# madsjulia/GeostatInversion.jl

Measured on AMD Instinct MI355X. Metric: randSVD GB/s + top-k singular-value rel-err, n=1e6 rank=256, higher is better.
Workload: dtype f64

## Files before the change

geostatinversion.jl_amd/build.py:

```python
import os
import shutil
import subprocess
import sys
from concurrent.futures import ThreadPoolExecutor

HERE = os.path.dirname(os.path.abspath(__file__))
CSRC = os.path.join(HERE, "csrc")
OBJ = os.path.join(HERE, "build")
LIB = os.path.join(HERE, "libgsi_hip.so")
SOURCES = ["gemm_f64.hip", "gemm_f64_gen1.hip", "syrk_f64.hip", "panel_lu_leaf.hip", "panel_lu_blocks.hip", "panel_lu_streamed.hip", "panel_lu_sharded.hip", "panel_qr.hip", "cholqr.hip", "lowrank_power.hip", "jacobi_svd.hip", "misc.hip", "lsqr_dev.hip", "pointcov_gemm.hip", "fft_cov.hip", "fft_gridcov_plan.hip", "fftrf_sample.hip", "fftrf_interp.hip", "pcga_forward.hip", "chol_saddle.hip",
           "hip_backend.hip", "hip_comm.hip", "pipeline.cpp", "api.cpp"]
HEADERS = ["backend.hpp", "hip_backend.hpp", "hip_common.hpp", "panel_lu_dev.hpp", "pipeline.hpp", "lsqr_state.hpp", "pointcov.hpp", "pointcov_gen.hpp", "host_staging.hpp", "gemm_f64_kernel.inc.hpp", "fft_line.hpp", "jacobi_sched.hpp", "fwd_plan.hpp", "fftrf_points.hpp", "saddle_host.hpp", "../../include/gsi_hip.h"]
CXXFLAGS = ["-O3", "-std=c++17", "-fPIC", "--offload-arch=gfx950", "-Wall", "-Wno-unused-function",
            "-Wno-unused-result", "-Wno-unused-value"]
RESOURCE_FLAG = "-Rpass-analysis=kernel-resource-usage"
_RES_KEYS = {"TotalSGPRs": "sgprs", "VGPRs": "vgprs", "AGPRs": "agprs", "ScratchSize [bytes/lane]": "scratch_bytes_per_lane",
             "Occupancy [waves/SIMD]": "occupancy_waves_per_simd", "SGPRs Spill": "sgpr_spills", "VGPRs Spill": "vgpr_spills",
             "LDS Size [bytes/block]": "lds_bytes_per_block", "Dynamic Stack": "dynamic_stack"}


def parse_resource_remarks(text):
    out, cur = {}, None
    for line in text.splitlines():
        if "remark:" not in line or "[-Rpass-analysis=kernel-resource-usage]" not in line:
            continue
        body = line.split("remark:", 1)[1].replace("[-Rpass-analysis=kernel-resource-usage]", "").strip()
        if ":" not in body:
            continue
        key, val = [x.strip() for x in body.rsplit(":", 1)]
        if key == "Function Name":
            cur = out.setdefault(val, {})
        elif cur is not None and key in _RES_KEYS:
            cur[_RES_KEYS[key]] = (val == "True") if key == "Dynamic Stack" else int(val)
    return out


def hipcc_version():
    r = subprocess.run([_hipcc(), "--version"], capture_output=True, text=True)
    lines = [ln.strip() for ln in r.stdout.splitlines() if ln.strip()]
    return "; ".join(lines[:2])


def kernel_resources():
    import json
    res = {}
    for src in SOURCES:
        if not src.endswith(".hip"):
            continue
        path = os.path.join(OBJ, src.replace(".", "_") + ".resources.json")
        if not os.path.exists(path):
            raise RuntimeError(f"{path} missing: run build() (it recompiles sources whose resource record is absent)")
        for name, r in json.load(open(path)).items():
            res[name] = dict(r, source=src)
    return res


def _hipcc():
    for cand in (shutil.which("hipcc"), "/opt/rocm/bin/hipcc"):
        if cand and os.path.exists(cand):
            return cand
    raise RuntimeError("hipcc not found: libgsi_hip.so cannot be built (there is no CPU fallback)")


# ... 54 lines not shown
```

geostatinversion.jl_amd/csrc/api.cpp:

```cpp
#include <cmath>
#include <cstdlib>
#include <cstring>
#include <memory>
#include <new>
#include <string>
#include <vector>
#include "../../include/gsi_hip.h"
#include "pipeline.hpp"
#include "pointcov.hpp"
#include "fftrf_points.hpp"

using namespace gsi;

struct gsi_ctx {
  Context c;
};
struct gsi_op {
  Operator op;
};
struct gsi_mat {
  gsi_ctx* ctx;
  Buf buf;
  int64_t rows, cols;
  int refs = 1;
// ... 952 lines not shown
  return guarded([&] {
    REQUIRE(ctx && Y && Q_out, "NULL argument");
    REQUIRE(m >= 1 && l >= 1 && l <= m, "qr_thinQ: need 1 <= l <= m (tall panel)");
    Backend* be = ctx->c.be.get();
    Buf P(be, (size_t)m * l), R(be, (size_t)l * l);
    be->upload2d(P.p, m, Y, m, m, l);
    {
      ScopedPhase ph(be, PH_QR);
      be->qr_thinQ(P.p, m, l, m, R.p);
    }
    be->download2d(Q_out, m, P.p, m, m, l);
    if (R_out) be->download2d(R_out, l, R.p, l, l, l);
    check_async_errors(ctx->c);
  });
}

int gsi_svd_tall(gsi_ctx* ctx, const double* W, int64_t n, int64_t l, double* V_out, double* S_out) {
  return guarded([&] {
    REQUIRE(ctx && W && V_out && S_out, "NULL argument");
    REQUIRE(n >= 1 && l >= 1 && l <= n, "svd_tall: need 1 <= l <= n");
    Backend* be = ctx->c.be.get();
    Buf Wd(be, (size_t)n * l), V(be, (size_t)n * l), S(be, (size_t)l);
    be->upload2d(Wd.p, n, W, n, n, l);
    svd_tall(ctx->c, Wd.p, n, l, -1, V.p, S.p);
    be->download2d(V_out, n, V.p, n, n, l);
    be->download2d(S_out, l, S.p, l, l, 1);
    check_async_errors(ctx->c);
  });
}

int gsi_gemm(gsi_ctx* ctx, int trans, int64_t m, int64_t l, int64_t k, double alpha, const double* A,
             int64_t lda, const double* B, int64_t ldb, double* C, int64_t ldc) {
  return guarded([&] {
    REQUIRE(ctx && A && B && C, "NULL argument");
    REQUIRE(m >= 1 && l >= 1 && k >= 1, "bad shape");
    const int64_t ar = trans ? k : m, ac = trans ? m : k;
    REQUIRE(lda >= ar && ldb >= k && ldc >= m, "leading dimension too small");
    Backend* be = ctx->c.be.get();
    Buf Ad(be, (size_t)ar * ac), Bd(be, (size_t)k * l), Cd(be, (size_t)m * l);
    be->upload2d(Ad.p, ar, A, lda, ar, ac);
    be->upload2d(Bd.p, k, B, ldb, k, l);
    if (trans) be->gemm_tn(m, l, k, alpha, Ad.p, ar, Bd.p, k, 0.0, Cd.p, m);
    else be->gemm_nn(m, l, k, alpha, Ad.p, ar, Bd.p, k, 0.0, Cd.p, m);
    be->download2d(C, ldc, Cd.p, m, m, l);
    check_async_errors(ctx->c);
  });
}

int gsi_gemm_view(gsi_ctx* ctx, int form, int trans, int64_t m, int64_t l, int64_t k, double alpha, double beta,
                  const double* A, int64_t lda, int64_t a_off, const double* B, int64_t ldb, int64_t b_off, double* C,
                  int64_t ldc, int64_t c_off, int64_t m_full, int64_t r0, int64_t* plan_out) {
  return guarded([&] {
    REQUIRE(ctx && A && C && plan_out, "NULL argument");
    REQUIRE(form >= 0 && form <= 3, "gemm_view: form is 0 (gemm), 1 (syrk upper), 2 (trmm upper) or 3 (NN row block)");
    REQUIRE(m >= 1 && l >= 1 && k >= 1, "bad shape");
    REQUIRE(form == 1 || B, "NULL argument");
    REQUIRE(form == 0 || (alpha == 1.0 && beta == 0.0), "gemm_view: forms 1 to 3 compute C = op(A) B (alpha 1, beta 0)");
    REQUIRE(form == 0 || !trans, "gemm_view: trans belongs to form 0");
    REQUIRE(form != 1 || m == l, "gemm_view: form 1 is the l x l product A'A (m == l)");
    REQUIRE(form != 3 || (r0 >= 0 && r0 + m <= m_full), "gemm_view: row block outside the full product");
    const bool tn = trans || form == 1;
    const int64_t ar = (form == 3) ? m_full : (tn ? k : m), ac = tn ? m : k;
    const int64_t crows = (form == 3) ? m_full : m;
    REQUIRE(lda >= ar && ldc >= crows && (form == 1 || ldb >= k), "leading dimension too small");
    REQUIRE(a_off >= 0 && b_off >= 0 && c_off >= 0, "negative offset");
    Backend* be = ctx->c.be.get();
    const size_t na = (size_t)a_off + (size_t)lda * (size_t)ac, nc = (size_t)c_off + (size_t)ldc * (size_t)l;
    const size_t nb = (form == 1) ? 1 : (size_t)b_off + (size_t)ldb * (size_t)l;
    Buf Ad(be, na), Bd(be, nb), Cd(be, nc);
    be->fill_bytes(Ad.p, 0xFF, na);
    be->fill_bytes(Bd.p, 0xFF, nb);
    be->upload2d(Ad.p + a_off, lda, A, ar, ar, ac);
    if (form != 1) be->upload2d(Bd.p + b_off, ldb, B, k, k, l);
    be->upload2d(Cd.p, (int64_t)nc, C, (int64_t)nc, (int64_t)nc, 1);
    be->gemm_view(form, trans != 0, m, l, k, alpha, Ad.p + a_off, lda, Bd.p + b_off, ldb, beta, Cd.p + c_off, ldc, m_full, r0,
                  plan_out);
    be->download2d(C, (int64_t)nc, Cd.p, (int64_t)nc, (int64_t)nc, 1);
    check_async_errors(ctx->c);
  });
}

namespace {
void pcga_params_impl(Context& c, const double* Zdev, int64_t n, int64_t K, const double* s, const double* X,
                      double delta, double* out) {
  Backend* be = c.be.get();
  Buf O(be, (size_t)n * (K + 3)), sv(be, (size_t)n), Xv(be, (size_t)n);
  be->upload2d(sv.p, n, s, n, n, 1);
  be->upload2d(Xv.p, n, X, n, n, 1);
  be->pcga_params(Zdev, n, K, sv.p, Xv.p, delta, O.p);
  be->download2d(out, n, O.p, n, n, K + 3);
}
void pcga_update_impl(Context& c, const double* Zdev, int64_t n, int64_t K, const double* X, double beta_bar,
                      const double* etas, int64_t nobs, const double* xi_bar, double* s_out) {
  Backend* be = c.be.get();
  Buf E(be, (size_t)nobs * K), xb(be, (size_t)nobs), w(be, (size_t)K), sd(be, (size_t)n), Xd(be, (size_t)n);
  be->upload2d(E.p, nobs, etas, nobs, nobs, K);
  be->upload2d(xb.p, nobs, xi_bar, nobs, nobs, 1);
  be->upload2d(Xd.p, n, X, n, n, 1);
  be->gemm_tn(K, 1, nobs, 1.0, E.p, nobs, xb.p, nobs, 0.0, w.p, K);
  be->scal_copy(n, beta_bar, Xd.p, sd.p);
  be->gemm_nn(n, 1, K, 1.0, Zdev, n, w.p, K, 1.0, sd.p, n);
  be->download2d(s_out, n, sd.p, n, n, 1);
}
}

int gsi_pcga_params(gsi_ctx* ctx, const double* Z, int64_t n, int64_t K, const double* s, const double* X,
                    double delta, double* out) {
  return guarded([&] {
    REQUIRE(ctx && Z && s && X && out, "NULL argument");
    REQUIRE(n >= 1 && K >= 1, "bad shape");
    Buf Zd(ctx->c.be.get(), (size_t)n * K);
// ... 315 lines not shown
```

geostatinversion.jl_amd/csrc/hip_backend.hip:

```cpp
#include <dlfcn.h>
#include <algorithm>
#include <cmath>
#include <cstdlib>
#include <cstring>
#include <mutex>
#include <map>
#include <memory>
#include <set>
#include <vector>
#include "hip_backend.hpp"
#include "hip_common.hpp"
#include "host_staging.hpp"
#include "fftrf_points.hpp"

namespace gsi {

namespace {

struct DevBuf {
  void* p = nullptr;
  size_t bytes = 0;
  bool pooled = false;
};

// ... 256 lines not shown
        HIP_CHECK(hipEventSynchronize(e1));
        float ms = 0.f;
        HIP_CHECK(hipEventElapsedTime(&ms, e0, e1));
        if (ms > 0.f) best[dir] = std::max(best[dir], (double)bytes / (ms * 1e-3) / 1e9);
      }
    *h2d_gbs = best[0];
    *d2h_gbs = best[1];
  }
  void upload2d_end(void* handle) override {
    if (!handle) return;
    try {
      static_cast<HostStager*>(handle)->end();
    } catch (const std::exception& e) {
      throw Error(GSI_ERR_HIP, e.what());
    }
  }
  void copy2d(double* dst, int64_t ldd, const double* src, int64_t lds, int64_t rows, int64_t cols) override {
    if (rows <= 0 || cols <= 0) return;
    bind();
    HIP_CHECK(hipMemcpy2DAsync(dst, ldd * sizeof(double), src, lds * sizeof(double), rows * sizeof(double),
                               cols, hipMemcpyDeviceToDevice, st_));
  }
  void fill_zero(double* p, size_t count) override {
    bind();
    HIP_CHECK(hipMemsetAsync(p, 0, count * sizeof(double), st_));
  }
  void sync() override {
    bind();
    HIP_CHECK(hipStreamSynchronize(st_));
    if (st2_) HIP_CHECK(hipStreamSynchronize(st2_));
  }

  void gemm_nn(int64_t m, int64_t l, int64_t k, double alpha, const double* A, int64_t lda, const double* B,
               int64_t ldb, double beta, double* C, int64_t ldc) override {
    bind();
    double* ws = gemm_ws(hipk::gemm_workspace_doubles(m, l, k));
    hipk::gemm_f64(st_, false, m, l, k, alpha, A, lda, B, ldb, beta, C, ldc, ws);
    check_launch("gemm_nn");
  }
  void gemm_nn_rowblock(int64_t m_full, int64_t r0, int64_t mb, int64_t l, int64_t k, const double* A, int64_t lda,
                        const double* B, int64_t ldb, double* C, int64_t ldc) override {
    bind();
    double* ws = gemm_ws(hipk::gemm_rowblock_workspace_doubles(m_full, mb, l, k));
    hipk::gemm_f64_nn_rowblock(st_, m_full, r0, mb, l, k, A, lda, B, ldb, C, ldc, ws);
    check_launch("gemm_nn_rowblock");
  }
  void gemm_tn(int64_t m, int64_t l, int64_t k, double alpha, const double* A, int64_t lda, const double* B,
               int64_t ldb, double beta, double* C, int64_t ldc) override {
    bind();
    double* ws = gemm_ws(hipk::gemm_workspace_doubles(m, l, k));
    hipk::gemm_f64(st_, true, m, l, k, alpha, A, lda, B, ldb, beta, C, ldc, ws);
    check_launch("gemm_tn");
  }
  void gemm_view(int form, bool trans, int64_t m, int64_t l, int64_t k, double alpha, const double* A, int64_t lda,
                 const double* B, int64_t ldb, double beta, double* C, int64_t ldc, int64_t m_full, int64_t r0,
                 int64_t* plan8) override {
    bind();
    hipk::GemmPlan p = {0, 0, 0, 0, 0, 0, 0, 0};
    if (form == 0) {
      double* ws = gemm_ws(hipk::gemm_workspace_doubles(m, l, k));
      hipk::gemm_f64(st_, trans, m, l, k, alpha, A, lda, B, ldb, beta, C, ldc, ws, &p);
    } else if (form == 1) {
      double* ws = gemm_ws(hipk::gemm_syrk_workspace_doubles(l, k));
      hipk::gemm_f64_syrk_upper(st_, l, k, A, lda, C, ldc, ws, &p);
    } else if (form == 2) {
      double* ws = gemm_ws(hipk::gemm_workspace_doubles(m, l, k));
      hipk::gemm_f64_trmm_upper(st_, m, l, k, A, lda, B, ldb, C, ldc, ws, &p);
    } else {
      double* ws = gemm_ws(hipk::gemm_rowblock_workspace_doubles(m_full, m, l, k));
      hipk::gemm_f64_nn_rowblock(st_, m_full, r0, m, l, k, A, lda, B, ldb, C, ldc, ws, &p);
    }
    check_launch("gemm_view");
    const int64_t out[8] = {p.nt, p.nchunks, p.xmode, p.wide, p.nsplit, p.persistent, p.grid_x, p.active};
    for (int i = 0; i < 8; ++i) plan8[i] = out[i];
  }
  void fill_bytes(double* p, int byte, size_t count) override {
    bind();
    HIP_CHECK(hipMemsetAsync(p, byte, count * sizeof(double), st_));
  }
  void gemm_nn_gridcov(int64_t m, int64_t l, int64_t k, const double* tab, int64_t nx, int64_t ny, int64_t roff,
                       int64_t koff, const double* B, int64_t ldb, double* C, int64_t ldc) override {
    bind();
    double* ws = gemm_ws(hipk::gemm_workspace_doubles(m, l, k));
    hipk::gemm_f64_gridcov(st_, m, l, k, tab, nx, ny, roff, koff, B, ldb, C, ldc, ws);
    check_launch("gemm_nn_gridcov");
  }

  void gemm_nn_pointcov(int64_t m, int64_t l, int64_t k, const double* pts, int d, int kind, double ell, double sigma2,
                        double nugget, int64_t roff, int64_t koff, const double* B, int64_t ldb, double* C,
                        int64_t ldc) override {
    bind();
    if (m <= 0 || l <= 0 || k <= 0) return;
    const int64_t npts = std::max(roff + m, koff + k);
    Scratch p4(this, (size_t)4 * npts);
    hipk::pointcov_pad_points(st_, pts, d, npts, hipk::pointcov_point_scale(kind, 1.0 / ell), p4.p);
    double* ws = gemm_ws(hipk::gemm_pointcov_workspace_doubles(m, l, k));
    Scratch xpack(this);
    const size_t xdoubles = hipk::gemm_pointcov_pack_doubles(m, l, k);
    if (xdoubles > 0) xpack.try_alloc(xdoubles);
    hipk::gemm_f64_pointcov(st_, m, l, k, p4.p, npts, d, kind, sigma2, nugget, roff, koff, B, ldb, C, ldc, ws, xpack.p);
    check_launch("gemm_nn_pointcov (in-loader generator)");
  }

  struct FftCov {
    int64_t N[3], M[3]; Scratch lam, W; int nb_max;
    explicit FftCov(HipBackend* be) : lam(be), W(be) {}
  };
  std::unique_ptr<FftCov> fftcov_new_plan(const int64_t N[3], int fftrf, bool* reembed, int* dims) {
    std::unique_ptr<FftCov> p(new FftCov(this));
    int64_t Mtot = 1;
    int d = 0;
    for (int a = 0; a < 3; ++a) { p->N[a] = 1; p->M[a] = 1; }
    *reembed = false;
    for (int a = 0; a < 3; ++a) {
      if (N[a] < 1) throw Error(GSI_ERR_ARG, "fft covariance: grid dimensions must be >= 1");
      if (N[a] == 1) continue;
      p->N[d] = N[a]; p->M[d] = hipk::fft_embed_size(N[a]);
      if (fftrf && p->M[d] != 2 * N[a]) *reembed = true;
      if (p->M[d] > 8192) throw Error(GSI_ERR_ARG, "fft covariance: at most 4096 grid points per axis (a line must fit LDS)");
      Mtot *= p->M[d];
      ++d;
    }
    if (Mtot >= ((int64_t)1 << 31))
// ... 485 lines not shown
  bool lowrank_tail(const double* Sm, int64_t lds, int64_t n, int64_t N, const double* G, const double* T, int64_t l,
                    int64_t K, double c, double* Z, int64_t ldz, double* Sv, double* scratch, size_t scratch_doubles) override {
    bind();
    if (!cholqr_gate(n, l) || l < 1 || l > 384 || l > N - 1 || K < 1 || K > l || N > 4096) return false;
    static const double ov_env = [] {
      const char* e = getenv("GSI_LOWRANK_TAIL_OVERLAP");
      if (e == nullptr || e[0] == 0) return -1.0;
      const double v = atof(e);
      return (v > 0.0 && v < 1.0) ? v : 0.0;
    }();
    static const int reserve = [] {
      const char* e = getenv("GSI_LOWRANK_TAIL_RESERVE_CUS");
      const int v = e ? atoi(e) : TAIL_RESERVE_CUS;
      return (v >= 8 && (v & 7) == 0) ? v : TAIL_RESERVE_CUS;
    }();
    const size_t Nl = ((size_t)N * l + 7) & ~(size_t)7, ll = ((size_t)l * l + 7) & ~(size_t)7;
    Scratch buf(this, 3 * Nl + 12 * ll);
    const int cap = std::max(8, ((ncus_ - reserve) / 8) * 8);
    int64_t nf = 0;
    if (ov_env != 0.0) {
      nf = (int64_t)((ov_env > 0.0 ? ov_env : TAIL_OVERLAP_FRACTION) * (double)n) / 128 * 128;
      if (nf >= n) nf = (n - 1) / 128 * 128;
    }
    double* A0 = buf.p;
    double* A1 = A0 + Nl;
    double* P = A1 + Nl;
    double* Gr[4];
    for (int i = 0; i < 4; ++i) Gr[i] = P + Nl + (size_t)i * ll;
    double* X[4];
    for (int i = 0; i < 4; ++i) X[i] = P + Nl + (size_t)(4 + i) * ll;
    double* R = P + Nl + 8 * ll;
    double* Rf = R + ll;
    double* U = Rf + ll;
    double* Mm = U + ll;
    size_t gmax = hipk::gemm_workspace_doubles(N, l, N);
    gmax = std::max(gmax, hipk::gemm_workspace_doubles(l, l, N));
    gmax = std::max(gmax, hipk::gemm_workspace_doubles(N, l, l));
    gmax = std::max(gmax, hipk::gemm_workspace_doubles(l, l, l));
    gmax = std::max(gmax, hipk::gemm_workspace_doubles(N, K, l));
    gmax = std::max(gmax, hipk::gemm_workspace_doubles(n, K, N));
    if (nf >= 128) {
      hipk::GemmPlan plan = {0, 0, 0, 0, 0, 0, 0, 0};
      const bool takes = hipk::gemm_f64_nn_capped(st_, nf, l, N, Sm, lds, A1, N, A1, nf, cap, true, &plan);
      if (!takes || (ov_env < 0.0 && plan.persistent == 0)) nf = 0;
    } else {
      nf = 0;
    }
    Scratch own(this, (nf > 0 && (scratch == nullptr || scratch_doubles < (size_t)nf * (size_t)l)) ? (size_t)nf * (size_t)l : 0);
    double* Yf = (nf > 0) ? (own.p != nullptr ? own.p : scratch) : nullptr;
    if (nf > 0) gmax = std::max(gmax, hipk::gemm_workspace_doubles(nf, K, l));
    double* ws = gemm_ws(gmax + 64);
    SideJoin side(this);
    auto round = [&](const double* M, int i, bool check) {
      hipk::gemm_f64(st_, false, N, l, N, 1.0, G, N, M, N, 0.0, P, N, ws);
      hipk::gemm_f64(st_, true, l, l, N, 1.0, M, N, P, N, 0.0, Gr[i], l, ws);
      (void)hipk::cq_gram_round(st_, Gr[i], l, X[i], check, flags_ + FLAG_CHOLQR);
    };
    phase_begin(PH_QR);
    HIP_CHECK(hipMemsetAsync(flags_ + FLAG_CHOLQR, 0, sizeof(int32_t), st_));
    hipk::scal_copy(st_, (int64_t)N * l, c, T, A0);
    round(A0, 0, false);
    hipk::gemm_f64(st_, false, N, l, l, 1.0, A0, N, X[0], l, 0.0, A1, N, ws);
    round(A1, 1, true);
    hipk::scal_copy(st_, (int64_t)N * l, c, P, A0);
    round(A0, 2, false);
    hipk::gemm_f64(st_, false, N, l, l, 1.0, A0, N, X[2], l, 0.0, A1, N, ws);
    round(A1, 3, true);
    check_launch("lowrank_tail");
    if (nf > 0) {
      side.fork();
      (void)hipk::gemm_f64_nn_capped(st2_, nf, l, N, Sm, lds, A1, N, Yf, nf, cap);
      check_launch("lowrank_tail (side product)");
    }
    if (read_flag(FLAG_CHOLQR) != 0) {
      side.join();
      phase_end(PH_QR);
      return false;
    }
    hipk::tri_product(st_, Gr[3], Gr[2], l, R);
    hipk::gemm_f64(st_, false, l, l, l, 1.0, R, l, X[1], l, 0.0, Rf, l, ws);
    phase_end(PH_QR);
    n_cholqr_ += 2;
    phase_begin(PH_SVD);
    svd_small(Rf, l, U, Sv);
    hipk::scale_cols_sqrt(st_, U, l, Sv, K);
    phase_end(PH_SVD);
    phase_begin(PH_SMALL_GEMM);
    hipk::gemm_f64(st_, false, l, K, l, 1.0, X[3], l, U, l, 0.0, Mm, l, ws);
    hipk::gemm_f64(st_, false, N, K, l, 1.0, A1, N, Mm, l, 0.0, A0, N, ws);
    if (nf > 0) {
      side.join();
      hipk::gemm_f64(st_, false, nf, K, l, 1.0, Yf, nf, Mm, l, 0.0, Z, ldz, ws);
      hipk::gemm_f64_nn_rowblock(st_, n, nf, n - nf, K, N, Sm, lds, A0, N, Z, ldz, ws);
      ++n_tail_overlaps_;
    } else {
      hipk::gemm_f64(st_, false, n, K, N, 1.0, Sm, lds, A0, N, 0.0, Z, ldz, ws);
    }
    if (K < l) HIP_CHECK(hipMemsetAsync(Z + (size_t)K * ldz, 0, sizeof(double) * ((size_t)(l - K - 1) * ldz + n), st_));
    check_launch("lowrank_tail");
    phase_end(PH_SMALL_GEMM);
    return true;
  }
  bool lowrank_power_step(const double* Sm, int64_t lds, int64_t n, int64_t N, const double* G, const double* T,
                          const int32_t* ipiv, const double* L, int64_t ldl, int64_t l, double c, double* Tn) override {
    bind();
    static const bool trace = (getenv("GSI_LOWRANK_POWER_TRACE") != nullptr);
    constexpr int64_t NSAMPLE = 256;
    constexpr int NPARTS = 128;
    constexpr double CHECK_MAX = 1e-8;
    if (l < 1 || l > 384 || N < 1 || N > 4096 || n < 2 * l || n >= ((int64_t)1 << 31)) return false;
    const int64_t ns = std::min<int64_t>(NSAMPLE, n - l), nchk = l + ns;
    auto up8 = [](int64_t x) { return (x + 7) & ~(int64_t)7; };
    const int64_t o_chk = up8(2 * l), o_sm = o_chk + up8(nchk), nr = o_sm + 2 * l, ldr = up8(nr);
    const size_t nidx = (size_t)(2 * ldr + nchk);
    const size_t ll = (size_t)up8(l * l), Nl = (size_t)up8(N * l);
    Scratch buf(this, 2 * ll + Nl + (size_t)ldr * (size_t)N + (size_t)ldr * (size_t)l + nidx + NPARTS + 2);
    double* Mp = buf.p;
    double* Ut = Mp + ll;
    double* C = Ut + ll;
    double* R = C + Nl;
    double* E = R + (size_t)ldr * N;
    int64_t* idx_dev = reinterpret_cast<int64_t*>(E + (size_t)ldr * l);
    double* part = reinterpret_cast<double*>(idx_dev + nidx);
    int32_t* verdict = reinterpret_cast<int32_t*>(part + NPARTS);
    const int64_t me = o_chk + nchk;
    size_t gmax = hipk::gemm_workspace_doubles(l, l, N);
    gmax = std::max(gmax, hipk::gemm_workspace_doubles(me, l, N));
    gmax = std::max(gmax, hipk::gemm_workspace_doubles(N, l, N));
    gmax = std::max(gmax, hipk::gemm_workspace_doubles(N, l, 2 * l));
    double* ws = gemm_ws(gmax + 64);
    struct Verdict { double parts[NPARTS]; int32_t v[4]; };
    if (pin_power_ == nullptr) HIP_CHECK(hipHostMalloc(&pin_power_, sizeof(Verdict), hipHostMallocDefault));
    hipk::lr_compose(st_, ipiv, flags_ + FLAG_LU_INFO, n, l, nchk, o_chk, o_sm, ldr, idx_dev, idx_dev + ldr, idx_dev + 2 * ldr, verdict);
    hipk::lr_gather_rows(st_, Sm, lds, N, idx_dev, idx_dev + ldr, nr, R, ldr);
    hipk::gemm_f64(st_, false, l, l, N, 1.0, R + o_chk, ldr, T, N, 0.0, Mp, l, ws);
    hipk::lr_solve_u(st_, L, ldl, Mp, l, c, Ut);
    hipk::lr_solve_c(st_, Ut, l, T, N, c, C);
    hipk::gemm_f64(st_, false, me, l, N, 1.0, R, ldr, C, N, 0.0, E, ldr, ws);
    hipk::lr_check_rows(st_, E + o_chk, ldr, L, ldl, idx_dev + 2 * ldr, nchk, l, part, NPARTS);
    hipk::gemm_f64(st_, false, N, l, N, 1.0, G, N, C, N, 0.0, Tn, N, ws);
    hipk::gemm_f64(st_, true, N, l, 2 * l, 1.0, R + o_sm, ldr, E, ldr, 1.0, Tn, N, ws);
    check_launch("lowrank_power_step");
    const Verdict* h = static_cast<const Verdict*>(pin_power_);
    HIP_CHECK(hipMemcpyAsync(pin_power_, part, sizeof(Verdict), hipMemcpyDeviceToHost, st_));
    HIP_CHECK(hipStreamSynchronize(st_));
    double mx = 0.0;
    bool finite = true;
    for (int p = 0; p < NPARTS; ++p) {
      if (!std::isfinite(h->parts[p])) finite = false;
      else mx = std::max(mx, h->parts[p]);
    }
    if (!finite) mx = INFINITY;
    if (trace) fprintf(stderr, "lowrank_power_step: n %lld N %lld l %lld, %lld moved rows, check max |(P S) C - L| = %.3e\n",
                       (long long)n, (long long)N, (long long)l, (long long)h->v[2], mx);
    if (h->v[0] != 0 || h->v[1] != 0) return false;
    return finite && mx <= CHECK_MAX;
  }
  static constexpr int64_t SPLIT_MAX_L1 = 192;
  struct SplitWs { int32_t* piv; int32_t* verdict1; int32_t* verdict2; int64_t* idx1; int64_t o_chk, o_sm, ldr; };
  static int64_t up8(int64_t x) { return (x + 7) & ~(int64_t)7; }
  SplitWs split_ws(int64_t l1) {
    SplitWs w;
    w.o_chk = up8(2 * l1); w.o_sm = w.o_chk + up8(l1); w.ldr = up8(w.o_sm + 2 * l1);
    grow(ws_split_, 2048 + sizeof(int64_t) * (size_t)(2 * up8(5 * SPLIT_MAX_L1 + 16) + SPLIT_MAX_L1));
    char* base = (char*)ws_split_.p;
    w.piv = (int32_t*)base;
    w.verdict1 = (int32_t*)(base + 1536 + 64);
    w.verdict2 = w.verdict1 + 4;
    w.idx1 = (int64_t*)(base + 2048);
    return w;
  }
  bool lu2_resident_ok() const {
    static const bool tall_first = (getenv("GSI_LU_TALL") != nullptr && getenv("GSI_LU_TALL")[0] == '1');
    return !tall_first && !lu2_lost_ && ranks_sharing_device_ <= 1;
  }
  bool lu2_takes(int64_t m, hipk::Lu2Work* w) {
    return lu2_resident_ok() && hipk::lu2_config(m, ncus_, &w->bs, &w->rpt, &w->grid) && lu2_fits(w->bs, w->rpt, w->grid);
  }
  bool lowrank_split_ok(int64_t n, int64_t N, int64_t l, int64_t l1) override {
    bind();
    if (l1 < 1 || l1 > SPLIT_MAX_L1 || l <= l1 || l > 2 * l1 || l - l1 < 8 || l > 384 || N < 1 || N > 4096 || n < 2 * l ||
        n >= ((int64_t)1 << 31))
      return false;
    hipk::Lu2Work w;
    return lu2_takes(n, &w) && lu2_takes(n - l1, &w);
  }
  void lowrank_split_schur(const double* Sm, int64_t lds, int64_t n, int64_t N, const double* T, const int32_t* ipiv1,
                           const double* P, int64_t ldp, int64_t l, int64_t l1, double c, double* Tt) override {
    bind();
    const int64_t l2 = l - l1;
    const SplitWs w = split_ws(l1);
    const size_t l1l = (size_t)up8(l1 * l), Nl1 = (size_t)up8(N * l1);
    Scratch buf(this, (size_t)up8(l1) * (size_t)N + 2 * l1l + 8 + Nl1);
    double* R = buf.p;
    double* Mp = R + (size_t)up8(l1) * N;
    double* Ut11 = Mp + l1l;
    double* U12 = Ut11 + (size_t)up8(l1 * l1);
    double* C1 = Mp + 2 * l1l + 8;
    size_t gmax = hipk::gemm_workspace_doubles(l1, l, N);
    gmax = std::max(gmax, hipk::gemm_workspace_doubles(N, l2, l1));
    double* ws = gemm_ws(gmax + 64);
    int64_t* src = w.idx1, * sub = w.idx1 + w.ldr, * chk = w.idx1 + 2 * w.ldr;
    hipk::lr_compose(st_, ipiv1, flags_ + FLAG_LU_INFO, n, l1, l1, w.o_chk, w.o_sm, w.ldr, src, sub, chk, w.verdict1);
    hipk::lr_pivots(st_, ipiv1, l1, 0, w.piv);
    hipk::lr_gather_rows(st_, Sm, lds, N, src + w.o_chk, sub + w.o_chk, l1, R, up8(l1));
    hipk::gemm_f64(st_, false, l1, l, N, 1.0, R, up8(l1), T, N, 0.0, Mp, l1, ws);
    hipk::lr_solve_u12(st_, P, ldp, Mp, l1, l, c, Ut11, U12);
    hipk::lr_solve_c(st_, Ut11, l1, T, N, c, C1);
    hipk::scal_copy(st_, N * l2, c, T + (size_t)N * l1, Tt);
    hipk::gemm_f64(st_, false, N, l2, l1, -1.0, C1, N, U12, l1, 1.0, Tt, N, ws);
    check_launch("lowrank_split_schur");
  }
  void lowrank_split_rows(double* P, int64_t ldp, int64_t n, int64_t l, int64_t l1) override {
    bind();
    (void)n;
    const int64_t l2 = l - l1;
    const SplitWs w = split_ws(l1);
    Scratch tmp(this, (size_t)(2 * l1) * (size_t)l2);
    hipk::lr_move_rows(st_, P + (size_t)l1 * ldp, ldp, l2, w.idx1, w.idx1 + w.ldr, w.verdict1, 2 * l1, tmp.p, 2 * l1, l1);
    check_launch("lowrank_split_rows");
  }
  void lowrank_split_join(double* P, int64_t ldp, int64_t n, int64_t l, int64_t l1, const int32_t* ipiv2,
                          int32_t** ipiv) override {
    bind();
    const int64_t l2 = l - l1;
    const SplitWs w = split_ws(l1);
    const int64_t ldr = up8(4 * l2);
    Scratch buf(this, (size_t)(2 * ldr + 8) + (size_t)(2 * l2) * (size_t)l1);
    int64_t* src = reinterpret_cast<int64_t*>(buf.p), * sub = src + ldr, * chk = sub + ldr;
    double* tmp = buf.p + 2 * ldr + 8;
    hipk::lr_compose(st_, ipiv2, flags_ + FLAG_LU_INFO, n - l1, l2, 0, 2 * l2, 2 * l2, ldr, src, sub, chk, w.verdict2);
    hipk::lr_pivots(st_, ipiv2, l2, l1, w.piv + l1);
    hipk::lr_move_rows(st_, P + l1, ldp, l1, src, sub, w.verdict2, 2 * l2, tmp, 2 * l2, 0);
    check_launch("lowrank_split_join");
    *ipiv = w.piv;
  }
  void lowrank_split_undo() override {
    bind();
    hipk::lr_forget_zero_pivot(st_, flags_ + FLAG_LU_INFO);
    check_launch("lowrank_split_undo");
  }
  void svd_small(double* G, int64_t l, double* U, double* S) override {
    bind();
    if (l > 5000) throw Error(GSI_ERR_ARG, "sketch width l = K+p > 5000 is not supported by the LDS-resident block Jacobi SVD");
    grow(ws_svd_, sizeof(double) * (l + 8) + 64 + sizeof(int32_t) * hipk::SVD_SCHED_INTS);
    hipk::SvdWork w;
    w.norms = (double*)ws_svd_.p;
    w.pairs = (int32_t*)((char*)ws_svd_.p + sizeof(double) * (l + 8) + 64);
    w.rotcount = flags_ + FLAG_SVD_ROTATIONS;
    const int sw = hipk::svd_small(st_, G, l, U, S, w);
    last_svd_sweeps_ = sw < 0 ? -sw : sw;
    if (sw < 0) ++n_svd_cap_hits_;
    check_launch("svd_small");
  }
  void chol_upper(double* B, int64_t j) override {
    bind();
    if (j > 2048) throw Error(GSI_ERR_ARG, "chol_upper: j too large");
    hipk::chol_upper(st_, B, j, flags_ + FLAG_CHOL_INFO);
    check_launch("chol_upper");
  }
  void trsm_right_upper(double* F, int64_t m, int64_t j, int64_t ldf, const double* C) override {
    bind();
    hipk::trsm_right_upper(st_, F, m, j, ldf, C);
// ... 509 lines not shown
```

geostatinversion.jl_amd/csrc/hip_common.hpp:

```cpp
#pragma once
#include <hip/hip_runtime.h>
#include <atomic>
#include <cstdint>
#include <cstddef>
#include "pointcov.hpp"

namespace gsi { struct FwdProduct; }

namespace gsi { namespace hipk {

inline bool first_use_on_this_device(std::atomic<uint64_t>& mask) {
  int dev = 0;
  if (hipGetDevice(&dev) != hipSuccess || dev < 0 || dev > 63) return true;
  const uint64_t bit = (uint64_t)1 << dev;
  return (mask.fetch_or(bit, std::memory_order_acq_rel) & bit) == 0;
}

struct GemmPlan { int64_t nt, nchunks, xmode, wide, nsplit, persistent, grid_x, active; };
size_t gemm_workspace_doubles(int64_t M, int64_t L, int64_t K);
void gemm_f64(hipStream_t st, bool transA, int64_t M, int64_t L, int64_t K, double alpha, const double* A,
              int64_t lda, const double* B, int64_t ldb, double beta, double* C, int64_t ldc, double* ws,
              GemmPlan* plan = nullptr);
bool gemm_f64_nn_capped(hipStream_t st, int64_t M, int64_t L, int64_t K, const double* A, int64_t lda, const double* B,
                        int64_t ldb, double* C, int64_t ldc, int max_grid, bool query_only = false, GemmPlan* plan = nullptr);
size_t gemm_rowblock_workspace_doubles(int64_t M_full, int64_t mb, int64_t L, int64_t K);
void gemm_f64_nn_rowblock(hipStream_t st, int64_t M_full, int64_t r0, int64_t mb, int64_t L, int64_t K, const double* A,
                          int64_t lda, const double* B, int64_t ldb, double* C, int64_t ldc, double* ws,
                          GemmPlan* plan = nullptr);
size_t gemm_syrk_workspace_doubles(int64_t l, int64_t m);
size_t syrk_upper_workspace_doubles(int64_t l, int64_t m);
bool syrk_full_from_upper(hipStream_t st, int64_t l, int64_t m, const double* Y, int64_t ld, double* G, int64_t ldg, double* ws);
bool trmm_upper_tall(hipStream_t st, int64_t m, int64_t l, const double* A, int64_t lda, const double* X, int64_t ldx, double* C,
                     int64_t ldc);
void gemm_f64_syrk_upper(hipStream_t st, int64_t l, int64_t m, const double* A, int64_t lda, double* C, int64_t ldc,
                         double* ws, GemmPlan* plan = nullptr);
void gemm_f64_trmm_upper(hipStream_t st, int64_t M, int64_t L, int64_t K, const double* A, int64_t lda, const double* B,
                         int64_t ldb, double* C, int64_t ldc, double* ws, GemmPlan* plan = nullptr);
void gemm_f64_gridcov(hipStream_t st, int64_t M, int64_t L, int64_t K, const double* tab, int64_t nx, int64_t ny,
                      int64_t roff, int64_t koff, const double* B, int64_t ldb, double* C, int64_t ldc, double* ws);

void gemm_f64_pointcov(hipStream_t st, int64_t M, int64_t L, int64_t K, const double* pts4, int64_t npts, int d, int kind,
                       double sigma2, double nugget, int64_t roff, int64_t koff, const double* B, int64_t ldb, double* C,
                       int64_t ldc, double* ws, double* xpack);
double pointcov_point_scale(int kind, double inv_ell);
bool gemm_f64_pointcov_wide(hipStream_t st, int64_t M, int64_t L, int64_t K, const double* pts4, int64_t npts, int d, int kind,
                            double sigma2, double nugget, int64_t roff, int64_t koff, const double* B, int64_t ldb, double* C,
                            int64_t ldc, double* ws, double* xpack);
size_t gemm_pointcov_workspace_doubles(int64_t M, int64_t L, int64_t K);
size_t gemm_pointcov_pack_doubles(int64_t M, int64_t L, int64_t K);
int gemm_choose_split(int64_t nwg, int64_t K);
void gemm_splitk_reduce(hipStream_t st, int64_t M, int64_t L, int nsplit, const double* slabs, double* C, int64_t ldc);
void pointcov_pad_points(hipStream_t st, const double* pts, int d, int64_t n, double scale, double* out4);
int64_t fft_embed_size(int64_t N);
size_t fft_plan_doubles(const int64_t M[3]);
void fft_spectrum(hipStream_t st, double* lam, double* part64, const int64_t M[3], double beta, int fftrf);
void fft_cos_matrix(hipStream_t st, double* out, int64_t rows, int64_t cols, int64_t period, bool weighted);
void fft_lines_layout(hipStream_t st, const double* nat, double* out, const int64_t M[3]);
void fft_spectrum_natural(hipStream_t st, double* lam, const int64_t M[3], double beta, int fftrf);
void fft_finish_plan(hipStream_t st, double* lam, double* part64, const int64_t M[3]);
void fft_plan_twiddles(hipStream_t st, double* lam, const int64_t M[3]);
void fft_lag_table(hipStream_t st, double* cp, double* cm, const int64_t N[3], int kind, const double inv_ell[3], double cs,
                   double sn, double sigma2);
void fft_even_odd_split(hipStream_t st, double* cp, double* cm, int64_t total);
void fft_sin_matrix(hipStream_t st, double* out, int64_t rows, int64_t cols, int64_t period);
void fft_subtract(hipStream_t st, double* a, const double* b, int64_t total);
void fft_finish_plan_lags(hipStream_t st, double* lam, const int64_t M[3], double nugget);
void fft_cov_apply(hipStream_t st, const int64_t N[3], const int64_t M[3], const double* lam, double2* W, int nb_max,
                   int64_t l, const double* X, int64_t ldx, double* Y, int64_t ldy);

struct FftrfGeom { int d; int64_t A[3], L[3], P[3]; int blue[3]; int64_t Mtot, n; };
void fftrf_geometry(int ndims, const int64_t* N, FftrfGeom* g);
size_t fftrf_plan_doubles(const FftrfGeom& g);
size_t fftrf_field_doubles(const FftrfGeom& g);
void fftrf_plan(hipStream_t st, const FftrfGeom& g, double* plan);
void fftrf_sample(hipStream_t st, const FftrfGeom& g, const double* plan, double* ws, int64_t fs, int nb, double k0, double dk,
                  double beta, double* dst, int64_t ldd, int64_t row0, int64_t nloc);
void fftrf_interp(hipStream_t st, int d, const int32_t* base, const double* frac, int64_t m, int64_t s1, int64_t s2,
                  const double* V, int64_t v_fs, int nb, double* dst, int64_t ldd);

constexpr int LU2_LEAF = 8;
constexpr int LU2_NB = 64;
// ... 166 lines not shown
```

Baseline: 1762.

## Add small-tile MFMA f64 GEMM for small products in low-rank power and QR

Adds a dedicated f64 GEMM kernel with 32x32 tiles and register prefetch, built on 16x16x4 f64 MFMA. It is used for small products (m up to 4096, l up to 384, small k) in the CholeskyQR tail, the power step and the split Schur paths. The aim is to cut launch and tiling overhead and raise occupancy on small operands, where the general GEMM's large tiles and workspace split waste work. It also exposes the kernel as gemm_view form 4 and adds an environment switch to disable it. The risk is lower throughput than the tuned general kernel on shapes near the thresholds.

```diff
diff --git a/geostatinversion.jl_amd/build.py b/geostatinversion.jl_amd/build.py
--- a/geostatinversion.jl_amd/build.py
+++ b/geostatinversion.jl_amd/build.py
@@ -8,7 +8,7 @@
 CSRC = os.path.join(HERE, "csrc")
 OBJ = os.path.join(HERE, "build")
 LIB = os.path.join(HERE, "libgsi_hip.so")
-SOURCES = ["gemm_f64.hip", "gemm_f64_gen1.hip", "syrk_f64.hip", "panel_lu_leaf.hip", "panel_lu_blocks.hip", "panel_lu_streamed.hip", "panel_lu_sharded.hip", "panel_qr.hip", "cholqr.hip", "lowrank_power.hip", "jacobi_svd.hip", "misc.hip", "lsqr_dev.hip", "pointcov_gemm.hip", "fft_cov.hip", "fft_gridcov_plan.hip", "fftrf_sample.hip", "fftrf_interp.hip", "pcga_forward.hip", "chol_saddle.hip",
+SOURCES = ["gemm_f64.hip", "gemm_f64_gen1.hip", "gemm_f64_small.hip", "syrk_f64.hip", "panel_lu_leaf.hip", "panel_lu_blocks.hip", "panel_lu_streamed.hip", "panel_lu_sharded.hip", "panel_qr.hip", "cholqr.hip", "lowrank_power.hip", "jacobi_svd.hip", "misc.hip", "lsqr_dev.hip", "pointcov_gemm.hip", "fft_cov.hip", "fft_gridcov_plan.hip", "fftrf_sample.hip", "fftrf_interp.hip", "pcga_forward.hip", "chol_saddle.hip",
            "hip_backend.hip", "hip_comm.hip", "pipeline.cpp", "api.cpp"]
 HEADERS = ["backend.hpp", "hip_backend.hpp", "hip_common.hpp", "panel_lu_dev.hpp", "pipeline.hpp", "lsqr_state.hpp", "pointcov.hpp", "pointcov_gen.hpp", "host_staging.hpp", "gemm_f64_kernel.inc.hpp", "fft_line.hpp", "jacobi_sched.hpp", "fwd_plan.hpp", "fftrf_points.hpp", "saddle_host.hpp", "../../include/gsi_hip.h"]
 CXXFLAGS = ["-O3", "-std=c++17", "-fPIC", "--offload-arch=gfx950", "-Wall", "-Wno-unused-function",
diff --git a/geostatinversion.jl_amd/csrc/api.cpp b/geostatinversion.jl_amd/csrc/api.cpp
--- a/geostatinversion.jl_amd/csrc/api.cpp
+++ b/geostatinversion.jl_amd/csrc/api.cpp
@@ -1028,11 +1028,14 @@
                   int64_t ldc, int64_t c_off, int64_t m_full, int64_t r0, int64_t* plan_out) {
   return guarded([&] {
     REQUIRE(ctx && A && C && plan_out, "NULL argument");
-    REQUIRE(form >= 0 && form <= 3, "gemm_view: form is 0 (gemm), 1 (syrk upper), 2 (trmm upper) or 3 (NN row block)");
+    REQUIRE(form >= 0 && form <= 4,
+            "gemm_view: form is 0 (gemm), 1 (syrk upper), 2 (trmm upper), 3 (NN row block) or 4 (small product, m_full = max workgroups)");
     REQUIRE(m >= 1 && l >= 1 && k >= 1, "bad shape");
     REQUIRE(form == 1 || B, "NULL argument");
-    REQUIRE(form == 0 || (alpha == 1.0 && beta == 0.0), "gemm_view: forms 1 to 3 compute C = op(A) B (alpha 1, beta 0)");
-    REQUIRE(form == 0 || !trans, "gemm_view: trans belongs to form 0");
+    REQUIRE(form == 0 || form == 4 || (alpha == 1.0 && beta == 0.0), "gemm_view: forms 1 to 3 compute C = op(A) B (alpha 1, beta 0)");
+    REQUIRE(form == 0 || form == 4 || !trans, "gemm_view: trans belongs to forms 0 and 4");
+    REQUIRE(form != 4 || (m_full >= 0 && m_full < ((int64_t)1 << 30) && (r0 == 0 || r0 == 32 || r0 == 64)),
+            "gemm_view: form 4 takes max workgroups (0: no cap) in m_full and the tile rows (0: the launcher's, 32, 64) in r0");
     REQUIRE(form != 1 || m == l, "gemm_view: form 1 is the l x l product A'A (m == l)");
     REQUIRE(form != 3 || (r0 >= 0 && r0 + m <= m_full), "gemm_view: row block outside the full product");
     const bool tn = trans || form == 1;
diff --git a/geostatinversion.jl_amd/csrc/gemm_f64_small.hip b/geostatinversion.jl_amd/csrc/gemm_f64_small.hip
--- /dev/null
+++ b/geostatinversion.jl_amd/csrc/gemm_f64_small.hip
@@ -0,0 +1,206 @@
+#include "hip_common.hpp"
+
+namespace gsi { namespace hipk {
+
+namespace {
+typedef double sp_double4 __attribute__((ext_vector_type(4)));
+constexpr int SP_THREADS = 256, SP_BN = 32, SP_BK = 32, SP_LDK = SP_BK + 2;
+constexpr int64_t SP_MAX_LD = (int64_t)1 << 20;
+
+template <int BM, bool TA>
+struct SpGeom {
+  static constexpr int WM = BM / 16, WN = 4 / WM, NACC = SP_BN / 16 / WN;
+  static constexpr int NA = BM * SP_BK / SP_THREADS, NB = SP_BN * SP_BK / SP_THREADS;
+  static constexpr int LDA_S = TA ? SP_LDK : BM + 16;
+  static constexpr int A_DOUBLES = TA ? BM * SP_LDK : SP_BK * (BM + 16);
+  static constexpr int B_DOUBLES = SP_BN * SP_LDK;
+  static constexpr int PF = BM == 32 ? 4 : 2;
+  static constexpr int KPASS = SP_THREADS / BM;
+};
+
+template <int NA, int NB>
+__device__ __forceinline__ void sp_load(double (&ra)[NA], double (&rb)[NB], const char* Ab, const char* Bb,
+                                        const uint32_t (&oa)[NA], const uint32_t (&ob)[NB]) {
+#pragma unroll
+  for (int i = 0; i < NA; ++i) ra[i] = *reinterpret_cast<const double*>(Ab + oa[i]);
+#pragma unroll
+  for (int i = 0; i < NB; ++i) rb[i] = *reinterpret_cast<const double*>(Bb + ob[i]);
+}
+
+template <int BM, bool TA, int NA, int NB>
+__device__ __forceinline__ void sp_load_tail(double (&ra)[NA], double (&rb)[NB], const char* Ab, const char* Bb, int64_t lda,
+                                             int64_t ldb, int mrem, int lrem, int krem) {
+  using G = SpGeom<BM, TA>;
+  const int t = threadIdx.x;
+#pragma unroll
+  for (int i = 0; i < NA; ++i) {
+    const int k = TA ? (t & 31) : t / BM + G::KPASS * i, r = min(TA ? (t >> 5) + 8 * i : t % BM, mrem - 1), kc = min(k, krem - 1);
+    const double v = *reinterpret_cast<const double*>(Ab + 8 * (TA ? kc + r * lda : r + kc * lda));
+    ra[i] = k < krem ? v : 0.0;
+  }
+#pragma unroll
+  for (int i = 0; i < NB; ++i) {
+    const int k = t & 31, c = min((t >> 5) + 8 * i, lrem - 1), kc = min(k, krem - 1);
+    const double v = *reinterpret_cast<const double*>(Bb + 8 * (kc + c * ldb));
+    rb[i] = k < krem ? v : 0.0;
+  }
+}
+
+template <int BM, bool TA, int NA, int NB>
+__device__ __forceinline__ void sp_stage(const double (&ra)[NA], const double (&rb)[NB], double* As, double* Bs) {
+  using G = SpGeom<BM, TA>;
+  const int t = threadIdx.x;
+  double* pa = TA ? As + (t >> 5) * SP_LDK + (t & 31) : As + (t / BM) * G::LDA_S + t % BM;
+  double* pb = Bs + (t >> 5) * SP_LDK + (t & 31);
+#pragma unroll
+  for (int i = 0; i < G::NA; ++i) pa[i * (TA ? 8 * SP_LDK : G::KPASS * G::LDA_S)] = ra[i];
+#pragma unroll
+  for (int i = 0; i < G::NB; ++i) pb[i * 8 * SP_LDK] = rb[i];
+}
+
+template <int BM, bool TA, int NACC>
+__device__ __forceinline__ void sp_mma(sp_double4 (&acc)[NACC], const double* as, const double* bs) {
+  using G = SpGeom<BM, TA>;
+  double a[SP_BK / 4], b[SP_BK / 4][NACC];
+#pragma unroll
+  for (int ks = 0; ks < SP_BK / 4; ++ks) {
+    a[ks] = as[TA ? ks * 4 : ks * 4 * G::LDA_S];
+#pragma unroll
+    for (int j = 0; j < NACC; ++j) b[ks][j] = bs[j * 16 * SP_LDK + ks * 4];
+  }
+#pragma unroll
+  for (int ks = 0; ks < SP_BK / 4; ++ks) {
+#pragma unroll
+    for (int j = 0; j < NACC; ++j) acc[j] = __builtin_amdgcn_mfma_f64_16x16x4f64(b[ks][j], a[ks], acc[j], 0, 0, 0);
+  }
+  __builtin_amdgcn_sched_group_barrier(0x100, SP_BK / 4 * (1 + NACC), 0);
+  __builtin_amdgcn_sched_group_barrier(0x008, SP_BK / 4 * NACC, 0);
+}
+
+template <int BM, bool TA>
+__global__ __launch_bounds__(SP_THREADS, 2) void gemm_f64_small_kernel(int M, int L, int K, double alpha,
+                                                                    const double* __restrict__ A, int64_t lda,
+                                                                    const double* __restrict__ B, int64_t ldb, double beta,
+                                                                    double* __restrict__ C, int64_t ldc, int tiles_m,
+                                                                    int ntiles) {
+  using G = SpGeom<BM, TA>;
+  __shared__ double As[2][G::A_DOUBLES];
+  __shared__ double Bs[2][G::B_DOUBLES];
+  const int t = threadIdx.x, lane = t & 63, wave = t >> 6;
+  const int wm = wave % G::WM, wn = wave / G::WM;
+  const int fi = lane & 15, fk = lane >> 4;
+  const int fa = TA ? (wm * 16 + fi) * SP_LDK + fk : fk * G::LDA_S + wm * 16 + fi;
+  const int fb = (wn * G::NACC * 16 + fi) * SP_LDK + fk;
+  const int nfull = K / SP_BK, krem = K % SP_BK;
+  const int64_t astep = TA ? (int64_t)8 * SP_BK : (int64_t)8 * SP_BK * lda, bstep = (int64_t)8 * SP_BK;
+
+  for (int tile = blockIdx.x; tile < ntiles; tile += gridDim.x) {
+    const int row0 = (tile % tiles_m) * BM, col0 = (tile / tiles_m) * SP_BN;
+    const int mrem = M - row0, lrem = L - col0;
+    const char* Ab = reinterpret_cast<const char*>(TA ? A + (int64_t)row0 * lda : A + row0);
+    const char* Bb = reinterpret_cast<const char*>(B + (int64_t)col0 * ldb);
+    uint32_t oa[G::NA], ob[G::NB];
+#pragma unroll
+    for (int i = 0; i < G::NA; ++i)
+      oa[i] = TA ? (uint32_t)(8 * ((t & 31) + min((t >> 5) + 8 * i, mrem - 1) * lda))
+                 : (uint32_t)(8 * (min(t % BM, mrem - 1) + (t / BM + G::KPASS * i) * lda));
+#pragma unroll
+    for (int i = 0; i < G::NB; ++i) ob[i] = (uint32_t)(8 * ((t & 31) + min((t >> 5) + 8 * i, lrem - 1) * ldb));
+    sp_double4 acc[G::NACC];
+#pragma unroll
+    for (int j = 0; j < G::NACC; ++j) acc[j] = sp_double4{0.0, 0.0, 0.0, 0.0};
+    if (nfull > 0) {
+      double ra[G::PF][G::NA], rb[G::PF][G::NB];
+#pragma unroll
+      for (int d = 0; d < G::PF; ++d) {
+        const int j = min(d, nfull - 1);
+        sp_load(ra[d], rb[d], Ab + j * astep, Bb + j * bstep, oa, ob);
+        __builtin_amdgcn_sched_barrier(0);
+      }
+      const int nmain = nfull / G::PF * G::PF;
+      for (int kt0 = 0; kt0 < nmain; kt0 += G::PF) {
+#pragma unroll
+        for (int d = 0; d < G::PF; ++d) {
+          const int cur = d & 1;
+          sp_stage<BM, TA>(ra[d], rb[d], As[cur], Bs[cur]);
+          const int j = min(kt0 + d + G::PF, nfull - 1);
+          sp_load(ra[d], rb[d], Ab + j * astep, Bb + j * bstep, oa, ob);
+          __builtin_amdgcn_sched_barrier(0);
+          __syncthreads();
+          sp_mma<BM, TA>(acc, As[cur] + fa, Bs[cur] + fb);
+          __builtin_amdgcn_sched_barrier(0);
+        }
+      }
+#pragma unroll
+      for (int d = 0; d < G::PF - 1; ++d) {
+        if (nmain + d < nfull) {
+          sp_stage<BM, TA>(ra[d], rb[d], As[d & 1], Bs[d & 1]);
+          __syncthreads();
+          sp_mma<BM, TA>(acc, As[d & 1] + fa, Bs[d & 1] + fb);
+        }
+      }
+    }
+    if (krem > 0) {
+      double ra[G::NA], rb[G::NB];
+      sp_load_tail<BM, TA>(ra, rb, Ab + nfull * astep, Bb + nfull * bstep, lda, ldb, mrem, lrem, krem);
+      sp_stage<BM, TA>(ra, rb, As[nfull & 1], Bs[nfull & 1]);
+      __syncthreads();
+      sp_mma<BM, TA>(acc, As[nfull & 1] + fa, Bs[nfull & 1] + fb);
+    }
+    __syncthreads();
+    const int r = wm * 16 + fi;
+    if (r < mrem) {
+#pragma unroll
+      for (int j = 0; j < G::NACC; ++j) {
+#pragma unroll
+        for (int q = 0; q < 4; ++q) {
+          const int c = (wn * G::NACC + j) * 16 + fk + 4 * q;
+          if (c < lrem) {
+            double* p = C + (int64_t)(row0 + r) + (int64_t)(col0 + c) * ldc;
+            double v = alpha * acc[j][q];
+            if (beta != 0.0) v += beta * *p;
+            *p = v;
+          }
+        }
+      }
+    }
+  }
+}
+
+template <int BM, bool TA>
+void sp_launch(hipStream_t st, int M, int L, int K, double alpha, const double* A, int64_t lda, const double* B, int64_t ldb,
+               double beta, double* C, int64_t ldc, int max_workgroups, GemmPlan* plan) {
+  const int tiles_m = (M + BM - 1) / BM, ntiles = tiles_m * ((L + SP_BN - 1) / SP_BN);
+  const int grid = (max_workgroups > 0 && max_workgroups < ntiles) ? max_workgroups : ntiles;
+  if (plan) *plan = GemmPlan{BM / 16, 1, 0, 0, 1, grid < ntiles ? 1 : 0, grid, ntiles};
+  hipLaunchKernelGGL((gemm_f64_small_kernel<BM, TA>), dim3(grid), dim3(SP_THREADS), 0, st, M, L, K, alpha, A, lda, B, ldb, beta, C,
+                     ldc, tiles_m, ntiles);
+}
+}
+
+bool gemm_f64_small_ok(int64_t M, int64_t L, int64_t K, int64_t lda, int64_t ldb) {
+  return M >= 1 && L >= 1 && K >= 1 && M <= 65536 && L <= 65536 && K <= ((int64_t)1 << 24) && lda < SP_MAX_LD && ldb < SP_MAX_LD &&
+         ((M + 31) / 32) * ((L + SP_BN - 1) / SP_BN) <= ((int64_t)1 << 24);
+}
+
+int gemm_f64_small_rows(int64_t M, int64_t L) {
+  (void)M; (void)L;
+  return 32;
+}
+
+bool gemm_f64_small(hipStream_t st, bool transA, int64_t M, int64_t L, int64_t K, double alpha, const double* A, int64_t lda,
+                    const double* B, int64_t ldb, double beta, double* C, int64_t ldc, int max_workgroups, GemmPlan* plan,
+                    int tile_rows) {
+  if (!gemm_f64_small_ok(M, L, K, lda, ldb)) return false;
+  const int bm = (tile_rows == 32 || tile_rows == 64) ? tile_rows : gemm_f64_small_rows(M, L);
+  if (bm == 64) {
+    if (transA) sp_launch<64, true>(st, (int)M, (int)L, (int)K, alpha, A, lda, B, ldb, beta, C, ldc, max_workgroups, plan);
+    else sp_launch<64, false>(st, (int)M, (int)L, (int)K, alpha, A, lda, B, ldb, beta, C, ldc, max_workgroups, plan);
+  } else {
+    if (transA) sp_launch<32, true>(st, (int)M, (int)L, (int)K, alpha, A, lda, B, ldb, beta, C, ldc, max_workgroups, plan);
+    else sp_launch<32, false>(st, (int)M, (int)L, (int)K, alpha, A, lda, B, ldb, beta, C, ldc, max_workgroups, plan);
+  }
+  return true;
+}
+
+}}
diff --git a/geostatinversion.jl_amd/csrc/hip_backend.hip b/geostatinversion.jl_amd/csrc/hip_backend.hip
--- a/geostatinversion.jl_amd/csrc/hip_backend.hip
+++ b/geostatinversion.jl_amd/csrc/hip_backend.hip
@@ -332,6 +332,22 @@
     hipk::gemm_f64(st_, true, m, l, k, alpha, A, lda, B, ldb, beta, C, ldc, ws);
     check_launch("gemm_tn");
   }
+  static bool small_product_takes(bool trans, int64_t m, int64_t l, int64_t k) {
+    (void)trans;
+    if (m > 4096 || l > 384) return false;
+    return k <= 384 || (k <= 1024 && l > 160 && m * l <= 1216 * 320);
+  }
+  void small_product(bool trans, int64_t m, int64_t l, int64_t k, double alpha, const double* A, int64_t lda, const double* B,
+                     int64_t ldb, double beta, double* C, int64_t ldc, double* ws, int max_workgroups = 0) {
+    static const bool off = [] {
+      const char* e = getenv("GSI_NO_SMALL_PRODUCT");
+      return e != nullptr && e[0] == '1';
+    }();
+    if (!off && small_product_takes(trans, m, l, k) &&
+        hipk::gemm_f64_small(st_, trans, m, l, k, alpha, A, lda, B, ldb, beta, C, ldc, max_workgroups))
+      return;
+    hipk::gemm_f64(st_, trans, m, l, k, alpha, A, lda, B, ldb, beta, C, ldc, ws);
+  }
   void gemm_view(int form, bool trans, int64_t m, int64_t l, int64_t k, double alpha, const double* A, int64_t lda,
                  const double* B, int64_t ldb, double beta, double* C, int64_t ldc, int64_t m_full, int64_t r0,
                  int64_t* plan8) override {
@@ -346,9 +362,12 @@
     } else if (form == 2) {
       double* ws = gemm_ws(hipk::gemm_workspace_doubles(m, l, k));
       hipk::gemm_f64_trmm_upper(st_, m, l, k, A, lda, B, ldb, C, ldc, ws, &p);
-    } else {
+    } else if (form == 3) {
       double* ws = gemm_ws(hipk::gemm_rowblock_workspace_doubles(m_full, m, l, k));
       hipk::gemm_f64_nn_rowblock(st_, m_full, r0, m, l, k, A, lda, B, ldb, C, ldc, ws, &p);
+    } else {
+      if (!hipk::gemm_f64_small(st_, trans, m, l, k, alpha, A, lda, B, ldb, beta, C, ldc, (int)m_full, &p, (int)r0))
+        throw Error(1 , "gemm_view: form 4 does not take these operands");
     }
     check_launch("gemm_view");
     const int64_t out[8] = {p.nt, p.nchunks, p.xmode, p.wide, p.nsplit, p.persistent, p.grid_x, p.active};
@@ -940,19 +959,19 @@
     double* ws = gemm_ws(gmax + 64);
     SideJoin side(this);
     auto round = [&](const double* M, int i, bool check) {
-      hipk::gemm_f64(st_, false, N, l, N, 1.0, G, N, M, N, 0.0, P, N, ws);
-      hipk::gemm_f64(st_, true, l, l, N, 1.0, M, N, P, N, 0.0, Gr[i], l, ws);
+      small_product(false, N, l, N, 1.0, G, N, M, N, 0.0, P, N, ws);
+      small_product(true, l, l, N, 1.0, M, N, P, N, 0.0, Gr[i], l, ws);
       (void)hipk::cq_gram_round(st_, Gr[i], l, X[i], check, flags_ + FLAG_CHOLQR);
     };
     phase_begin(PH_QR);
     HIP_CHECK(hipMemsetAsync(flags_ + FLAG_CHOLQR, 0, sizeof(int32_t), st_));
     hipk::scal_copy(st_, (int64_t)N * l, c, T, A0);
     round(A0, 0, false);
-    hipk::gemm_f64(st_, false, N, l, l, 1.0, A0, N, X[0], l, 0.0, A1, N, ws);
+    small_product(false, N, l, l, 1.0, A0, N, X[0], l, 0.0, A1, N, ws);
     round(A1, 1, true);
     hipk::scal_copy(st_, (int64_t)N * l, c, P, A0);
     round(A0, 2, false);
-    hipk::gemm_f64(st_, false, N, l, l, 1.0, A0, N, X[2], l, 0.0, A1, N, ws);
+    small_product(false, N, l, l, 1.0, A0, N, X[2], l, 0.0, A1, N, ws);
     round(A1, 3, true);
     check_launch("lowrank_tail");
     if (nf > 0) {
@@ -966,7 +985,7 @@
       return false;
     }
     hipk::tri_product(st_, Gr[3], Gr[2], l, R);
-    hipk::gemm_f64(st_, false, l, l, l, 1.0, R, l, X[1], l, 0.0, Rf, l, ws);
+    small_product(false, l, l, l, 1.0, R, l, X[1], l, 0.0, Rf, l, ws);
     phase_end(PH_QR);
     n_cholqr_ += 2;
     phase_begin(PH_SVD);
@@ -974,8 +993,8 @@
     hipk::scale_cols_sqrt(st_, U, l, Sv, K);
     phase_end(PH_SVD);
     phase_begin(PH_SMALL_GEMM);
-    hipk::gemm_f64(st_, false, l, K, l, 1.0, X[3], l, U, l, 0.0, Mm, l, ws);
-    hipk::gemm_f64(st_, false, N, K, l, 1.0, A1, N, Mm, l, 0.0, A0, N, ws);
+    small_product(false, l, K, l, 1.0, X[3], l, U, l, 0.0, Mm, l, ws);
+    small_product(false, N, K, l, 1.0, A1, N, Mm, l, 0.0, A0, N, ws);
     if (nf > 0) {
       side.join();
       hipk::gemm_f64(st_, false, nf, K, l, 1.0, Yf, nf, Mm, l, 0.0, Z, ldz, ws);
@@ -1021,13 +1040,13 @@
     if (pin_power_ == nullptr) HIP_CHECK(hipHostMalloc(&pin_power_, sizeof(Verdict), hipHostMallocDefault));
     hipk::lr_compose(st_, ipiv, flags_ + FLAG_LU_INFO, n, l, nchk, o_chk, o_sm, ldr, idx_dev, idx_dev + ldr, idx_dev + 2 * ldr, verdict);
     hipk::lr_gather_rows(st_, Sm, lds, N, idx_dev, idx_dev + ldr, nr, R, ldr);
-    hipk::gemm_f64(st_, false, l, l, N, 1.0, R + o_chk, ldr, T, N, 0.0, Mp, l, ws);
+    small_product(false, l, l, N, 1.0, R + o_chk, ldr, T, N, 0.0, Mp, l, ws);
     hipk::lr_solve_u(st_, L, ldl, Mp, l, c, Ut);
     hipk::lr_solve_c(st_, Ut, l, T, N, c, C);
-    hipk::gemm_f64(st_, false, me, l, N, 1.0, R, ldr, C, N, 0.0, E, ldr, ws);
+    small_product(false, me, l, N, 1.0, R, ldr, C, N, 0.0, E, ldr, ws);
     hipk::lr_check_rows(st_, E + o_chk, ldr, L, ldl, idx_dev + 2 * ldr, nchk, l, part, NPARTS);
-    hipk::gemm_f64(st_, false, N, l, N, 1.0, G, N, C, N, 0.0, Tn, N, ws);
-    hipk::gemm_f64(st_, true, N, l, 2 * l, 1.0, R + o_sm, ldr, E, ldr, 1.0, Tn, N, ws);
+    small_product(false, N, l, N, 1.0, G, N, C, N, 0.0, Tn, N, ws);
+    small_product(true, N, l, 2 * l, 1.0, R + o_sm, ldr, E, ldr, 1.0, Tn, N, ws);
     check_launch("lowrank_power_step");
     const Verdict* h = static_cast<const Verdict*>(pin_power_);
     HIP_CHECK(hipMemcpyAsync(pin_power_, part, sizeof(Verdict), hipMemcpyDeviceToHost, st_));
@@ -1092,11 +1111,11 @@
     hipk::lr_compose(st_, ipiv1, flags_ + FLAG_LU_INFO, n, l1, l1, w.o_chk, w.o_sm, w.ldr, src, sub, chk, w.verdict1);
     hipk::lr_pivots(st_, ipiv1, l1, 0, w.piv);
     hipk::lr_gather_rows(st_, Sm, lds, N, src + w.o_chk, sub + w.o_chk, l1, R, up8(l1));
-    hipk::gemm_f64(st_, false, l1, l, N, 1.0, R, up8(l1), T, N, 0.0, Mp, l1, ws);
+    small_product(false, l1, l, N, 1.0, R, up8(l1), T, N, 0.0, Mp, l1, ws);
     hipk::lr_solve_u12(st_, P, ldp, Mp, l1, l, c, Ut11, U12);
     hipk::lr_solve_c(st_, Ut11, l1, T, N, c, C1);
     hipk::scal_copy(st_, N * l2, c, T + (size_t)N * l1, Tt);
-    hipk::gemm_f64(st_, false, N, l2, l1, -1.0, C1, N, U12, l1, 1.0, Tt, N, ws);
+    small_product(false, N, l2, l1, -1.0, C1, N, U12, l1, 1.0, Tt, N, ws);
     check_launch("lowrank_split_schur");
   }
   void lowrank_split_rows(double* P, int64_t ldp, int64_t n, int64_t l, int64_t l1) override {
diff --git a/geostatinversion.jl_amd/csrc/hip_common.hpp b/geostatinversion.jl_amd/csrc/hip_common.hpp
--- a/geostatinversion.jl_amd/csrc/hip_common.hpp
+++ b/geostatinversion.jl_amd/csrc/hip_common.hpp
@@ -27,6 +27,11 @@
 void gemm_f64_nn_rowblock(hipStream_t st, int64_t M_full, int64_t r0, int64_t mb, int64_t L, int64_t K, const double* A,
                           int64_t lda, const double* B, int64_t ldb, double* C, int64_t ldc, double* ws,
                           GemmPlan* plan = nullptr);
+bool gemm_f64_small_ok(int64_t M, int64_t L, int64_t K, int64_t lda, int64_t ldb);
+int gemm_f64_small_rows(int64_t M, int64_t L);
+bool gemm_f64_small(hipStream_t st, bool transA, int64_t M, int64_t L, int64_t K, double alpha, const double* A, int64_t lda,
+                    const double* B, int64_t ldb, double beta, double* C, int64_t ldc, int max_workgroups = 0,
+                    GemmPlan* plan = nullptr, int tile_rows = 0);
 size_t gemm_syrk_workspace_doubles(int64_t l, int64_t m);
 size_t syrk_upper_workspace_doubles(int64_t l, int64_t m);
 bool syrk_full_from_upper(hipStream_t st, int64_t l, int64_t m, const double* Y, int64_t ld, double* G, int64_t ldg, double* ws);
```

New measurement: 1778, median of 6. No clear change (+0.9%).
